# smann95/mpmc

Measured on AMD Instinct MI355X. Metric: MC steps/sec (polarizable, 4096 atoms), higher is better.
Workload: dtype f64; 1 GPU; PCN-61 cell + 416 BSSP H2, 4096 atoms (2016 frozen), polarizable, Jacobi x4, rc 8 A, FH4; energy() incremental (bit-identical to full); n_atoms=4096, n_polarizable=3264, n_atoms_final=4096, n_polarizable_final=3264, walkers=1, parallelism=1 independent walkers, 1 per GPU, collective=none (single walker, no launcher), rccl_ranks=1

## Files before the change

mpmc_amd/csrc/engine.hip:

```cpp
#include "../../include/mpmc_hip.h"

#include <dlfcn.h>
#include <hip/hip_runtime.h>
#include <hip/hip_ext.h>
#include <rccl/rccl.h>

#include <algorithm>
#include <cmath>
#include <cstdarg>
#include <cstdio>
#include <cstring>
#include <functional>
#include <map>
#include <memory>
#include <tuple>
#include <utility>
#include <ctime>
#include <numeric>
#include <atomic>
#include <string>
#include <vector>

#include "device_common.h"
#include "kernels_pair.h"
#include "kernels_disp.h"
#include "kernels_at.h"
#include "kernels_crystal.h"
#include "kernels_vdw.h"
#include "kernels_polar.h"
#include "kernels_exact.h"
#include "kernels_gs.h"
#include "kernels_gs_chain.h"
#include "kernels_resident.h"
#include "kernels_symv.h"
#include "kernels_coef.h"
#include "kernels_volume.h"
#include "kernels_cavity.h"

using namespace mpmc;

static thread_local std::string g_err;
static std::atomic<int> g_ctx_on_device[64];

static int fail(const char *fmt, ...) {
    char buf[1024];
    va_list ap;
    va_start(ap, fmt);
    vsnprintf(buf, sizeof(buf), fmt, ap);
    va_end(ap);
    g_err = buf;
    return -1;
}

#define HIPCHK(expr)                                                                           \
    do {                                                                                       \
        hipError_t e_ = (expr);                                                                \
        if (e_ != hipSuccess) return fail("MPMC_HIP: %s failed: %s (%s:%d)", #expr, hipGetErrorString(e_), \
                                          __FILE__, __LINE__);                                 \
    } while (0)

extern "C" const char *mpmc_hip_last_error(void) { return g_err.c_str(); }
extern "C" int mpmc_hip_abi_version(void) { return MPMC_HIP_ABI_VERSION; }
extern "C" int mpmc_hip_device_count(void) {
    int n = 0;
    if (hipGetDeviceCount(&n) != hipSuccess) return 0;
    return n;
}

template <typename T, bool kPinned>
class HipBuffer {
  public:
    HipBuffer() = default;
    HipBuffer(HipBuffer &&o) noexcept : p_(std::exchange(o.p_, nullptr)), n_(std::exchange(o.n_, 0)) {}
    ~HipBuffer() { reset(); }
    hipError_t alloc(size_t count, unsigned host_flags = hipHostMallocDefault) {
        reset();
        void *p = nullptr;
        hipError_t e;
        if constexpr (kPinned)
            e = hipHostMalloc(&p, count * sizeof(T), host_flags);
        else
            e = hipMalloc(&p, count * sizeof(T));
        if (e == hipSuccess) p_ = static_cast<T *>(p), n_ = count;
        return e;
    }
    void reset() {
        if (p_) {
            if constexpr (kPinned)
                hipHostFree(p_);
            else
// ... 154 lines not shown
    int gs_build_fork = 1;
    int gs_side_waves = 0;
    int rank_view_side = 1;
    int gs_fold_upper = 1;
    int gs_fold_finish = 1;
    int rank_late = 1;
    int resident = 1;
    int res_fold = 16;
    int res_side = 0;
    int sweep_alternate = 1;
    int sweep_nt = -1;
    int sweep_split = -1;
    int fuse_moves = 1;
    int gs_fuse_moves = 1;
    int fuse_field = 1;
    int fuse_recip = 1;
    int split_record = 1;
    int side_moves = 1;
    int res_stamps = 0;
    int sweep_ablate = 0;
    int res_fault = 0;
    int gs_stamps = 0;
    int inv_stamps = 0;
    int gs_ablate = 0;
    int gs_fault_sweep = 0;
    int graph = 0;
};

struct CallState {
    bool do_polar = false;
    bool gs_mode = false;
    bool exact = false;
    bool two_streams = false;
    bool plain_launches = false;
    DirtyBlocks dirty_blocks;
    bool pair_part_valid_before = false;
    bool moves_deferred = false;
    bool moves_in_pair = false;
    bool side_carry = false;
    MoveList side_moves;
    MoveList pair_moves;
    MoveList side_apply;
    bool side_applied = false;
    bool coef_job_valid = false;
    bool coef_job_fork = false;
    CoefJob coef_job;
    bool build_join_pending = false;
    bool rank_on_side = false;
    int gs_sweeps = 0;
    bool gs_used[2] = {false, false};
    std::function<void()> enqueue_side;
    std::function<void()> publish_early;
    bool published = false;
    bool recip_fused = false;
    int recip_chunks = 0;
    int pair_rows_to_sum = 0;
    unsigned res_zero_mask = 0;
    bool split = false;
    bool resident = false;
    bool spec_rank = false;
    bool timed = false;
    int iterations = 0, iter_success = 0;
};

struct TileSum {
    DevBuf<double> part;
    bool valid = false;
};

struct mpmc_hip_ctx {
    int device = 0;
    int num_cus = 256;
    int max_atoms = 0, max_npad = 0;
    int n = 0, npad = 0;
    EngineOptions opt;
    CallState call;
    mpmc_hip_params par;
    bool have_params = false, have_box = false, have_atoms = false;
    double basis[3][3], recip[3][3];
    double pbc_cutoff_in = 0.0, cutoff = 0.0, volume = 0.0, ewald_alpha = 0.0, polar_ewald_alpha = 0.0;
    bool box_ortho = false;
    double coord_max = 0.0;
    unsigned long long config_rev = 1;
    unsigned long long energy_calls = 0;
    bool in_flight = false;
    HipStream stream;
    HipStream stream2;
    HipStream stream3;
    HipEvent ev_fork, ev_join;
    HipEvent ev_rank;
    HipEvent ev_bfork, ev_bjoin;
    HipEvent ev_order;
    DevBuf<double> d_x, d_y, d_z, d_q, d_alpha, d_eps, d_sig, d_molmass;
    DevBuf<int> d_mol, d_flags;
    MoveList pending;
    std::vector<int> dirty_atoms;
    bool all_dirty = true;
    bool staged_copies = false;
    bool main_writes = false;
    SweepView view[2];
    DevBuf<double> d_es, d_mu, d_efind, d_efchg, d_tmp3;
    DevBuf<unsigned long long> d_errmax;
    bool have_polar_result = false;
    SweepView *result_view = nullptr;
    const double *result_mu = nullptr;
    bool results_scattered = true;
// ... 75 lines not shown
    DevBuf<KVec> d_kvec;
    int nk = 0;
    bool kvec_valid = false;
    int kvec_kmax = -1;
    DevBuf<double2> d_sfpart;
    bool recip_part_valid = false;
    DevBuf<double> d_recipsum;
    bool self_valid = false;
    double self_alpha = 0.0;
    DevBuf<KVecF> d_kvecf;
    DevBuf<double2> d_sf;
    int nkf = 0;
    double kvecf_alpha = -1.0;
    int kvecf_kmax = -1;
    bool kvecf_valid = false;
    DevBuf<double> d_rank;
    DevBuf<double> d_rankpart;
    DevBuf<double> d_rank_used;
    DevBuf<unsigned int> d_rankcnt;
    std::vector<double> rank_saved;
    bool perm_ranked = false;
    bool rank_used_valid = false;
    bool force_host_rank = false;
    unsigned long long spec_redos = 0;
    int n_valid = 0;
    int next_mol = 0;
    std::vector<char> slot_valid;
    std::vector<char> slot_polar;
    std::vector<std::pair<int, int>> holes;
    std::vector<int> lrc_dirty_atoms;
    int n_mol_uploaded = 0;
    bool edited = false;
    bool order_stale = false;
    bool resident_off = false;
    long resident_retry_at = 0;
    long resident_backoff = 0;
    bool force_multi_launch = false;
    bool res_attr_set = false;
    unsigned long long resident_calls = 0, resident_fallbacks = 0;
    int graph_mode = 0;
    StepGraph sg;
    int eligible_streak = 0;
    unsigned long long graph_launches = 0;
    double graph_update_s = 0.0, graph_launch_s = 0.0;
    PinnedBuf<int> h_dirty;
    PinnedBuf<double> h_stage;
    size_t stage_used = 0;
    DevBuf<double> d_delta;
    DevBuf<double> d_res;
    PinnedBuf<double> h_res;
    double *h_res_dev = nullptr;
    PinnedBuf<double> h_res2;
    double *h_res2_dev = nullptr;
    PinnedBuf<unsigned long long> h_err;
    PinnedBuf<unsigned> h_gserr;
    PinnedBuf<int> h_order;
    PinnedBuf<double> h_rank;
    PinnedBuf<int> h_perm;
    PinnedBuf<int> h_slotmap;
    std::vector<HipEvent> ev_pool;
    size_t ev_next = 0;
    std::vector<TimeRec> recs;
    HipEvent ev_first, ev_last;
    bool timed = false;
    double host_enqueue_s = 0.0, host_wait_s = 0.0;
};

static DevAtoms dev_atoms(const mpmc_hip_ctx *c) {
    DevAtoms a;
    a.x = c->d_x;
    a.y = c->d_y;
    a.z = c->d_z;
    a.q = c->d_q;
    a.alpha = c->d_alpha;
    a.eps = (c->disp_on || c->rdc_order || c->vdw_on) ? c->d_zero : c->d_eps;
    a.sig = (c->disp_on || c->rdc_order || c->vdw_on) ? c->d_zero : c->d_sig;
    a.molmass = c->d_molmass;
    a.mol = c->d_mol;
    a.flags = c->d_flags;
    a.n = c->n;
    a.npad = c->npad;
    return a;
}

static DevBox dev_box(const mpmc_hip_ctx *c) {
    DevBox b;
    for (int p = 0; p < 3; ++p)
        for (int q = 0; q < 3; ++q) {
            b.b[p][q] = c->basis[p][q];
            b.rb[p][q] = c->recip[p][q];
        }
    b.cutoff = c->cutoff;
    b.volume = c->volume;
    for (int p = 0; p < 3; ++p)
        for (int q = 0; q < 3; ++q) {
            b.fb[p][q] = (float)c->basis[p][q];
            b.frb[p][q] = (float)c->recip[p][q];
        }
    b.rc2_pre = (float)((c->cutoff + 0.01) * (c->cutoff + 0.01));
    b.screen64 = (c->coord_max > kScreen32MaxCoord || !(c->coord_max == c->coord_max)) ? 1 : 0;
    double smax = 0.0, rmax = 0.0;
    for (int q = 0; q < 3; ++q) {
        smax = std::max(smax, std::fabs(c->recip[0][q]) + std::fabs(c->recip[1][q]) + std::fabs(c->recip[2][q]));
        for (int p = 0; p < 3; ++p) rmax = std::max(rmax, std::fabs(c->recip[p][q]));
    }
    const float tie32 = (float)(1.25 * 11.0 * 0x1p-13 * smax);
// ... 246 lines not shown
    HIPCHK(c->d_sig.alloc(np));
    HIPCHK(c->d_molmass.alloc(np));
    HIPCHK(c->d_mol.alloc(np));
    HIPCHK(c->d_flags.alloc(np));
    HIPCHK(c->d_es.alloc(3 * np));
    HIPCHK(c->d_mu.alloc(3 * np));
    HIPCHK(c->d_efind.alloc(3 * np));
    HIPCHK(c->d_efchg.alloc(3 * np));
    HIPCHK(c->d_tmp3.alloc(3 * np));
    HIPCHK(c->d_rank.alloc(np));
    HIPCHK(c->d_rank_used.alloc(np));
    HIPCHK(c->d_rankcnt.alloc(np));
    HIPCHK(c->d_errmax.alloc(256));
    for (SweepView &v : c->view) {
        v.cap = (int)np;
        HIPCHK(v.d_idx.alloc(np));
        HIPCHK(v.d_slot.alloc(np));
        HIPCHK(v.px.alloc(np));
        HIPCHK(v.py.alloc(np));
        HIPCHK(v.pz.alloc(np));
        HIPCHK(v.palpha.alloc(np));
        HIPCHK(v.pflags.alloc(np));
        HIPCHK(v.es.alloc(3 * np));
        HIPCHK(v.mu0.alloc(3 * np));
        HIPCHK(v.mu1.alloc(3 * np));
        HIPCHK(v.munew.alloc(3 * np));
        HIPCHK(v.mupub.alloc(kGsMaxLag * (3 * np + 192)));
        c->gs_qoff = (int)(3 * np + 192);
        HIPCHK(v.y.alloc(3 * np));
        HIPCHK(v.efind.alloc(3 * np));
        HIPCHK(v.tmu0.alloc(3 * np));
        HIPCHK(v.efchg.alloc(3 * np));
        HIPCHK(v.rrms.alloc(np));
        HIPCHK(v.gsflags.alloc(16));
        HIPCHK(hipMemsetAsync(v.gsflags, 0, 16 * sizeof(unsigned), c->stream));
        HIPCHK(v.energy_part.alloc(2 * (np / 64 + 1)));
        for (double *p : {v.mu0.get(), v.mu1.get(), v.munew.get(), v.y.get(), v.efind.get(), v.efchg.get(), v.es.get()})
            HIPCHK(hipMemsetAsync(p, 0, 3 * np * sizeof(double), c->stream));
        HIPCHK(hipMemsetAsync(v.rrms, 0, np * sizeof(double), c->stream));
    }
    const size_t ntile = np / 64;
    HIPCHK(c->d_pairpart.alloc(ntile * ntile * kPairChannels));
    HIPCHK(c->lrc.part.alloc(ntile * ntile));
    HIPCHK(c->d_rankpart.alloc(ntile * ntile));
    const size_t nchunk_max = std::max<size_t>(1, np / 64) + 16;
    HIPCHK(c->d_fieldpart.alloc(nchunk_max * 3 * np));
    HIPCHK(c->d_res.alloc(R_COUNT));
    HIPCHK(c->h_res.alloc(R_COUNT + 1, hipHostMallocMapped));
    c->h_res[R_COUNT] = 0.0;
    HIPCHK(hipHostGetDevicePointer((void **)&c->h_res_dev, c->h_res, 0));
    HIPCHK(c->h_res2.alloc(R_COUNT + 1, hipHostMallocMapped));
    memset(c->h_res2, 0, (R_COUNT + 1) * sizeof(double));
    HIPCHK(hipHostGetDevicePointer((void **)&c->h_res2_dev, c->h_res2, 0));
    HIPCHK(c->h_err.alloc(1));
    HIPCHK(c->h_gserr.alloc(2));
    HIPCHK(c->h_rank.alloc(np));
    HIPCHK(c->h_perm.alloc(np));
    HIPCHK(c->h_slotmap.alloc(np));
    HIPCHK(c->h_dirty.alloc(kMaxDirty));
    HIPCHK(c->h_stage.alloc(3 * 4096));
    c->ev_pool.resize(2 * 512);
    for (auto &e : c->ev_pool) HIPCHK(hipEventCreate(e.out()));
    HIPCHK(hipEventCreate(c->ev_first.out()));
    HIPCHK(hipEventCreate(c->ev_last.out()));
    HIPCHK(hipMemsetAsync(c->d_res, 0, R_COUNT * sizeof(double), c->stream));
    HIPCHK(hipStreamSynchronize(c->stream));
    if (device < 64) ++g_ctx_on_device[device];
    *out = owner.release();
    return 0;
}

static void graph_destroy(mpmc_hip_ctx *c);

extern "C" void mpmc_hip_destroy(mpmc_hip_ctx *c) {
    if (!c) return;
    if (getenv("MPMC_HIP_HOST_PROFILE") && c->energy_calls)
        fprintf(stderr, "MPMC_HIP host profile: %llu energy() calls (%llu as graph), enqueue %.1f us, wait %.1f us per call\n",
                c->energy_calls, c->graph_launches, 1e6 * c->host_enqueue_s / c->energy_calls,
                1e6 * c->host_wait_s / c->energy_calls);
    if (getenv("MPMC_HIP_HOST_PROFILE") && c->graph_launches)
        fprintf(stderr, "MPMC_HIP graph steps: node updates %.1f us, launch %.1f us per step\n",
                1e6 * c->graph_update_s / c->graph_launches, 1e6 * c->graph_launch_s / c->graph_launches);
    hipSetDevice(c->device);
    hipStreamSynchronize(c->stream);
    hipStreamSynchronize(c->stream2);
    hipStreamSynchronize(c->stream3);
    graph_destroy(c);
    if (c->device < 64) --g_ctx_on_device[c->device];
    delete c;
}

static void positions_unknown(mpmc_hip_ctx *c) {
    c->pair_part_valid = c->field_part_valid = c->disp.valid = c->rdc.valid = c->at.valid = false;
    c->rep.valid = c->vdw.valid = false;
}
static void params_or_grid_changed(mpmc_hip_ctx *c) {
    c->pair_part_valid = c->field_part_valid = c->disp.valid = c->rdc.valid = false;
    c->rep.valid = c->vdw.valid = false;
}
static void box_changed(mpmc_hip_ctx *c) {
    c->lrc.valid = c->disp_lrc.valid = c->rdc_static.valid = c->rep_lrc.valid = c->vdw_lrc.valid = false;
    c->cav_pos_valid = c->cav_occ_valid = false;
    c->cav_open = -1;
}
static void atoms_replaced(mpmc_hip_ctx *c) {
    c->lrc.valid = c->disp.valid = c->disp_lrc.valid = c->at.valid = c->rdc.valid = c->rdc_static.valid = false;
// ... 1791 lines not shown
                hipGraph_t graph = nullptr;
                ok = (hipStreamEndCapture(c->stream, &graph) == hipSuccess) && rc == 0 && graph != nullptr;
                if (ok) ok = graph_finish_capture(c, graph);
                else if (graph) hipGraphDestroy(graph);
            }
            if (ok) {
                c->sg.valid = true;
                c->sg.rev = c->config_rev;
                c->sg.iterations = c->call.iterations;
                c->sg.result_view = c->result_view;
                c->sg.result_mu = c->result_mu;
                c->sg.psweep = c->psweep;
                c->sg.energy_part = c->energy_part;
                c->sg.energy_nt = c->energy_nt;
                c->sg.recip_chunks = c->call.recip_chunks;
                c->sg.res_zero_mask = c->call.res_zero_mask;
                c->sg.pair_rows_to_sum = c->call.pair_rows_to_sum;
                HIPCHK(hipGraphLaunch(c->sg.exec, c->stream));
                ++c->graph_launches;
                issued = true;
            } else {
                (void)hipGetLastError();
                graph_destroy(c);
                c->opt.graph = 0;
                c->pending = saved;
                c->call = CallState();
                collect_dirty_blocks(c);
            }
        }
    } else {
        c->eligible_streak = 0;
    }
    if (!issued && enqueue_direct(c)) return -1;
    c->staged_copies = false;
    c->main_writes = false;
    clock_gettime(CLOCK_MONOTONIC, &ts1);
    c->host_enqueue_s += (ts1.tv_sec - ts0.tv_sec) + 1e-9 * (ts1.tv_nsec - ts0.tv_nsec);
    c->dirty_atoms.clear();
    c->all_dirty = false;
    c->in_flight = true;
    return 0;
}

static int wait_sequence(volatile double *seq, double want, hipStream_t stream) {
    for (unsigned long long spins = 0; spins < 2000000000ull; ++spins) {
        if (*seq == want) return 0;
        if ((spins & 0xfffffull) == 0xfffffull && hipStreamQuery(stream) != hipErrorNotReady) break;
        __builtin_ia32_pause();
    }
    HIPCHK(hipStreamSynchronize(stream));
    return 0;
}

static int wait_record(mpmc_hip_ctx *c) {
    const double want = (double)c->energy_calls;
    if (wait_sequence(c->h_res + R_COUNT, want, c->stream)) return -1;
    return c->call.split ? wait_sequence(c->h_res2 + R_COUNT, want, c->stream2) : 0;
}

static int repeat_call(mpmc_hip_ctx *c, bool &flag) {
    flag = true;
    begin_call(c);
    const int rc = enqueue_direct(c);
    flag = false;
    return rc ? -1 : wait_record(c);
}

extern "C" int mpmc_hip_energy_end(mpmc_hip_ctx *c, mpmc_hip_result *out) {
    if (!c || !out) return fail("MPMC_HIP: energy: null argument");
    if (!c->in_flight) return fail("MPMC_HIP: energy_end: no evaluation in flight");
    c->in_flight = false;
    memset(out, 0, sizeof(*out));
    const mpmc_hip_params &P = c->par;
    timespec ts1, ts2;
    clock_gettime(CLOCK_MONOTONIC, &ts1);
    if (wait_record(c)) return -1;
    if (c->call.spec_rank && c->h_res[R_GS_ERR] == 0.0 && c->h_res[R_RANKCHG] != 0.0) {
        ++c->spec_redos;
        if (repeat_call(c, c->force_host_rank)) return -1;
    }
    if (c->call.resident && c->h_res[R_GS_ERR] != 0.0) {
        ++c->resident_fallbacks;
        c->resident_off = true;
        c->resident_backoff = c->resident_backoff ? std::min(2 * c->resident_backoff, 1L << 20) : 4096;
        c->resident_retry_at = (long)c->energy_calls + c->resident_backoff;
        c->view[0].resP_armed = false;
        if (repeat_call(c, c->force_multi_launch)) return -1;
    }
    clock_gettime(CLOCK_MONOTONIC, &ts2);
    c->host_wait_s += (ts2.tv_sec - ts1.tv_sec) + 1e-9 * (ts2.tv_nsec - ts1.tv_nsec);
    const bool do_polar = c->call.do_polar, timed_call = c->call.timed;
    const int polar_iterations = c->call.iterations;
    const int iter_success = c->call.exact ? (c->h_res[R_RRMS] != 0.0 ? 1 : 0) : c->call.iter_success;
    if (c->call.exact) {
        c->chol_done = true;
        c->chol_failed = iter_success != 0;
    }
    const int gs_err = (int)c->h_res[R_GS_ERR];
    c->h_gserr[0] = gs_err & 1;
    c->h_gserr[1] = (gs_err >> 1) & 1;
    const bool gs_timeout = gs_err != 0;
    if (gs_timeout) {
        unsigned dbg[8] = {0};
        const SweepView &gv = c->view[c->h_gserr[1] ? 1 : 0];
        hipMemcpy(dbg, gv.gsflags, sizeof(dbg), hipMemcpyDeviceToHost);
        return fail("MPMC_HIP: persistent Gauss-Seidel kernel gave up waiting on a hand-off (spin limit) in view %d: "
                    "workgroup %u thread %u addr-lo 0x%x; mu_new-lo 0x%x",
                    c->h_gserr[1] ? 1 : 0, dbg[2], dbg[3], dbg[4], (unsigned)((unsigned long long)gv.mupub.get() & 0xffffffffu));
    }
    HIPCHK(hipGetLastError());
    c->timed = timed_call;
    c->stage_used = 0;

    double r[R_COUNT];
    for (int k = 0; k < R_COUNT; ++k) r[k] = (c->call.split && ((kSideSlots >> k) & 1u)) ? c->h_res2[k] : c->h_res[k];
    const double rd = c->disp_on     ? (r[R_RD_PAIR] + r[R_LRC]) + (r[R_DISP] + r[R_DISP_LRC])
                      : c->rdc_order ? (r[R_RD_PAIR] + r[R_LRC]) + ((r[R_DISP] + r[R_RDC_SELF]) + r[R_DISP_LRC])
                      : c->vdw_on    ? (r[R_RD_PAIR] + r[R_LRC]) + (r[R_DISP] + r[R_DISP_LRC])
                                     : r[R_RD_PAIR] + r[R_LRC];
    const double real = r[R_ES_REAL] - r[R_ES_INTRA];
    const bool ewald = !P.rd_only && !P.wolf;
    const double recip = ewald ? r[R_RECIP] * (4.0 * kPI / c->volume) : 0.0;
    const double self = ewald ? r[R_SELF] : 0.0;
    const double coul = P.rd_only ? 0.0 : real + recip + self;
    const double upol = do_polar ? r[R_UPOL] : 0.0;
    out->rd_energy = rd;
    out->es_real = P.rd_only ? 0.0 : real;
    out->es_recip = recip;
    out->es_self = self;
    out->coulombic_energy = coul;
    out->polarization_energy = upol;
    out->energy = rd + coul + upol;
    c->three_body = c->at_on ? r[R_AT] : 0.0;
    if (c->at_on) out->energy += c->three_body;
    c->vdw_energy = (c->vdw_on && !P.rd_only) ? ((r[R_VDW] - c->vdw_e_iso) + 0.0) + r[R_VDW_LRC] : 0.0;
    if (c->vdw_on) out->energy += c->vdw_energy;
    c->vdw_terms[0] = (c->vdw_on && !P.rd_only) ? r[R_VDW] : 0.0;
    c->vdw_terms[1] = (c->vdw_on && !P.rd_only) ? c->vdw_e_iso : 0.0;
    c->vdw_terms[2] = (c->vdw_on && !P.rd_only) ? r[R_VDW_LRC] : 0.0;
    c->vdw_terms[3] = c->vdw_on ? r[R_DISP] : 0.0;
    c->vdw_terms[4] = c->vdw_on ? r[R_DISP_LRC] : 0.0;
    c->close_contacts = c->autoreject_scale != 0.0 ? (long long)r[R_CONTACTS] : 0;
    out->dipole_rrms = (do_polar && !c->call.exact) ? r[R_RRMS] : 0.0;
    out->volume = c->volume;
    out->cutoff = c->cutoff;
    out->ewald_alpha = c->ewald_alpha;
    out->polar_ewald_alpha = c->polar_ewald_alpha;
    out->polar_iterations = polar_iterations;
    out->iter_success = iter_success;
    out->n_atoms = c->n_valid;
    out->status = std::isfinite(out->energy) ? 0 : 1;
    return 0;
}

extern "C" int mpmc_hip_download_dipoles(mpmc_hip_ctx *c, double *mu, double *ef_static, double *ef_induced,
                                         double *ef_induced_change) {
    if (!c || !c->have_atoms) return fail("MPMC_HIP: download_dipoles: no configuration");
    if (!c->have_polar_result) return fail("MPMC_HIP: download_dipoles: no polarization energy evaluated yet");
    HIPCHK(hipSetDevice(c->device));
    if (ensure_static_field(c)) return -1;
    if (complete_pending_sweep(c)) return -1;
    if (!c->results_scattered) {
        SweepView *V = c->result_view;
        hipLaunchKernelGGL(scatter_results_kernel, dim3((c->npad + 255) / 256), dim3(256), 0, c->stream, c->npad,
                           V->d_slot, c->result_mu, V->efind, V->efchg, c->d_mu, c->d_efind, c->d_efchg);
        HIPCHK(hipStreamSynchronize(c->stream));
        c->results_scattered = true;
    }
// ... 425 lines not shown
```

mpmc_amd/csrc/engine_polar.inc:

```
static constexpr bool kSweepSplitAuto = false;

static int launch_coef_job(mpmc_hip_ctx *c, const DevBox &bx) {
    if (!c->call.coef_job_valid) return 0;
    c->call.coef_job_valid = false;
    const CoefJob &cj = c->call.coef_job;
    hipLaunchKernelGGL(update_coef_moves_kernel, dim3(cj.nt, cj.dm.n), dim3(64), 0, c->stream, cj.pa, bx, cj.damp, cj.dm,
                       cj.ntld, cj.C, cj.m, cj.gx, cj.gy, cj.gz, cj.slot_of_atom, cj.px, cj.py, cj.pz);
    if (c->call.coef_job_fork) hipEventRecord(c->ev_fork, c->stream);
    return 0;
}

static int launch_field(mpmc_hip_ctx *c, const DevAtoms &a, const DevBox &bx) {
    const mpmc_hip_params &P = c->par;
    ScopedTimer t(c, T_FIELD);
    FieldParams fp;
    fp.wolf_alpha = P.polar_wolf_alpha;
    fp.cutoffterm = 0.0;
    const int ntile = c->npad / 64;
    int nchunk = std::max(1, std::min(ntile, 4096 / ntile));
    int chunk = round_up((c->npad + nchunk - 1) / nchunk, 64);
    nchunk = (c->npad + chunk - 1) / chunk;
    fp.chunk = chunk;
    const int mode = P.polar_ewald ? kFieldEwald : (!P.polar_wolf ? kFieldBare : (P.polar_wolf_alpha == 0.0 ? kFieldWolf0 : kFieldWolfA));
    const int key = mode * 1000003 + chunk;
// ... 298 lines not shown
                c->call.build_join_pending = true;
            }
            if (istamps) {
                --c->opt.inv_stamps;
                std::vector<unsigned long long> h(nwg * 4);
                HIPCHK(hipStreamSynchronize(st));
                HIPCHK(hipMemcpy(h.data(), istamps, h.size() * sizeof(unsigned long long), hipMemcpyDeviceToHost));
                unsigned long long t0 = ~0ull, t3 = 0;
                double ph[3] = {0, 0, 0}, phmax[3] = {0, 0, 0}, start_max = 0;
                int live = 0;
                for (size_t g = 0; g < nwg; ++g) {
                    if (!h[4 * g + 3]) continue;
                    t0 = std::min(t0, h[4 * g]);
                }
                for (size_t g = 0; g < nwg; ++g) {
                    if (!h[4 * g + 3]) continue;
                    ++live;
                    t3 = std::max(t3, h[4 * g + 3]);
                    start_max = std::max(start_max, (double)(h[4 * g] - t0) * 0.01);
                    for (int k = 0; k < 3; ++k) {
                        const double d = (double)(h[4 * g + k + 1] - h[4 * g + k]) * 0.01;
                        ph[k] += d;
                        phmax[k] = std::max(phmax[k], d);
                    }
                }
                fprintf(stderr, "INV_STAMPS waves %d, %d live workgroups of %zu (lists %d %d %d, full %d): span %.2f us, last start +%.2f us; "
                                "mean (max) us: loads %.2f (%.2f), expansion %.2f (%.2f), substitution %.2f (%.2f)\n",
                        waves, live, nwg, gb.inv.n, gb.own.n, nsingle, full ? 1 : 0, (double)(t3 - t0) * 0.01, start_max, ph[0] / std::max(live, 1),
                        phmax[0], ph[1] / std::max(live, 1), phmax[1], ph[2] / std::max(live, 1), phmax[2]);
            }
        }
        v.M_epoch = v.C_epoch;
        v.M_call = c->energy_calls;
    }
    if (want_matrix) {
        if (ensure_view_matrix(v)) return -1;
        if (can_update && v.A_valid) {
            if (nd > 0)
                hipLaunchKernelGGL(update_amatrix_kernel, dim3(v.nvpad / 128, nd), dim3(64), 0, st, pa, bx,
                                   c->par.polar_damp, dl, v.A, 3 * v.nvpad);
        } else {
            hipLaunchKernelGGL(build_amatrix_kernel, dim3(v.nvpad / 128, v.nvpad / kARows), dim3(64), 0, st, pa, bx,
                               c->par.polar_damp, v.A, 3 * v.nvpad);
            v.A_valid = true;
        }
    } else {
        v.A_valid = false;
    }
    return 0;
}

template <int MODE>
static int launch_sweep(mpmc_hip_ctx *c, SweepView &v, const DevBox &bx, const double *mu_in, double *out,
                        const SweepParams &sp, int timer_class, const double *mu_final = nullptr) {
    const int nvpad = v.nvpad, lda = 3 * nvpad;
    if (v.C_valid) {
        const int nt = std::max(1, (v.nv + kCoefTile - 1) / kCoefTile);
        if (ensure_coef_scratch(v, nt)) return -1;
        CoefFinish fin;
        fin.alpha = v.palpha;
        fin.flags = v.pflags;
        fin.mu_in = mu_in;
        fin.es = v.es;
        fin.ef_induced = v.efind;
        fin.out = out;
        fin.rrms = v.rrms;
        fin.errmax = c->d_errmax;
        fin.mu_final = mu_final;
        fin.energy_part = v.energy_part;
        fin.tmu0 = v.tmu0;
        fin.sp = sp;
        size_t half_plane = 0;
        {
            const int ntiles = nt * (nt + 1) / 2;
            const bool split = c->opt.sweep_split > 0 || (c->opt.sweep_split < 0 && kSweepSplitAuto && nt > 21 && ntiles < 8 * c->num_cus);
            half_plane = split ? 2 * (3 * (size_t)kCoefTile * nt) * (size_t)nt : 0;
            const dim3 g(split ? 16 * ((ntiles + 7) / 8) : ntiles), b(64 * kCoefWaves);
            const size_t tile_bytes = (size_t)nt * (nt + 1) / 2 * kCoefTile * kCoefTile * sizeof(double2);
            const bool sweep_nt = c->opt.sweep_nt > 0 || (c->opt.sweep_nt < 0 && tile_bytes > ((size_t)224 << 20));
            void (*kern)(const double2 *, int, int, const double *, const double *, const double *, const double *, DevBox,
                         double *, double *, int, size_t) =
                c->box_ortho ? (sweep_nt ? pair_sweep_kernel<1, 1> : pair_sweep_kernel<1, 0>)
                             : (sweep_nt ? pair_sweep_kernel<0, 1> : pair_sweep_kernel<0, 0>);
            if (split)
                kern = c->box_ortho ? (sweep_nt ? pair_sweep_kernel<1, 1, 0, 1> : pair_sweep_kernel<1, 0, 0, 1>)
                                    : (sweep_nt ? pair_sweep_kernel<0, 1, 0, 1> : pair_sweep_kernel<0, 0, 0, 1>);
            if (c->opt.sweep_ablate == 1) kern = pair_sweep_kernel<1, 0, 1>;
            if (c->opt.sweep_ablate == 2) kern = pair_sweep_kernel<1, 0, 2>;
            if (c->opt.sweep_ablate) half_plane = 0;
            HIPCHK(launch_timed(c, timer_class, kern, g, b, 0, c->stream, (const double2 *)v.C, nt, v.ntld,
                                (const double *)v.px, (const double *)v.py, (const double *)v.pz, mu_in, bx, v.Srow, v.Zcol,
                                c->opt.sweep_alternate ? (c->sweep_parity++ & 1) : 0, half_plane));
        }
        {
            ScopedTimer t2(c, T_OTHER);
            hipLaunchKernelGGL(pair_finish_kernel<MODE>, dim3(nt), dim3(64 * kCoefFinishGroups), 0, c->stream, nt, v.Srow,
                               v.Zcol, fin, half_plane);
        }
        c->energy_part = v.energy_part;
        c->energy_nt = nt;
        return 0;
    }
    c->energy_nt = 0;
    if (c->opt.symmetric && (nvpad >= 2048 || c->opt.symmetric > 1)) {
        if (ensure_sym_scratch(v)) return -1;
        {
            ScopedTimer t(c, timer_class);
            const dim3 g(nvpad / kSymChunkAtoms, nvpad / kSymRowAtoms);
            const int rev = (c->opt.sym_mode & 1) ? (c->sweep_parity++ & 1) : 0;
            if (c->opt.sym_mode & 2)
                hipLaunchKernelGGL(symv_kernel<1>, g, dim3(64), 0, c->stream, v.A, lda, nvpad, mu_in, v.Srow, v.Zcol, rev,
                                   v.nv);
            else
                hipLaunchKernelGGL(symv_kernel<0>, g, dim3(64), 0, c->stream, v.A, lda, nvpad, mu_in, v.Srow, v.Zcol, rev,
                                   v.nv);
        }
        ScopedTimer t2(c, T_OTHER);
        hipLaunchKernelGGL(symv_finish_kernel<MODE>, dim3(nvpad / 64), dim3(1024), 0, c->stream, nvpad, v.Srow, v.Zcol,
                           v.palpha, v.pflags, mu_in, v.es, v.efind, out, v.rrms, c->d_errmax, sp);
    } else {
        ScopedTimer t(c, timer_class);
        hipLaunchKernelGGL(sweep_kernel<MODE>, dim3(nvpad), dim3(64), 0, c->stream, v.A, lda, nvpad, v.palpha,
                           v.pflags, mu_in, v.es, v.efind, out, v.rrms, c->d_errmax, sp);
    }
    return 0;
}

static bool defer_last_sweep(const mpmc_hip_ctx *c, const SweepView &v) {
    const mpmc_hip_params &P = c->par;
    if (!c->opt.pair_coef || !v.C_valid) return false;
    if (P.polar_zodid || P.polar_gs || P.polar_gs_ranked || P.polar_palmo || P.polar_sor || P.polar_esor || P.polar_rrms)
        return false;
    if (P.polar_precision != 0.0 || P.polar_gamma != 1.0 || P.polar_max_iter < 2) return false;
    const int nt = std::max(1, (v.nv + kCoefTile - 1) / kCoefTile);
    return nt * (nt + 1) / 2 + nt > c->num_cus;
}

static int complete_pending_sweep(mpmc_hip_ctx *c) {
    if (c->psweep.sweeps.empty()) return 0;
    PendingSweep p;
    std::swap(p, c->psweep);
    HIPCHK(hipSetDevice(c->device));
    for (const PendingSweep::One &s : p.sweeps)
        if (launch_sweep<kSweepJacobi>(c, *p.view, p.bx, s.mu_in, s.mu_out, s.sp, T_SWEEP)) return -1;
    return 0;
}

static void (*chain_kernel_of(int ortho))(GsChain) { return ortho ? gs_chain_kernel<1> : gs_chain_kernel<0>; }

static bool gs_uses_chain(const mpmc_hip_ctx *c) { return c->opt.pair_coef != 0 && c->opt.persistent_gs != 0; }

struct GsFinishArgs {
    double w_new, w_old;
    int want_rrms, err_slot;
    double *mu_out;
};
static int launch_gs_sweep(mpmc_hip_ctx *c, SweepView &v, const DevAtoms &a, const DevBox &bx, const double *mu_old,
                           const GsFinishArgs *fin = nullptr, bool *finished = nullptr) {
    if (finished) *finished = false;
    const int nvpad = v.nvpad, lda = 3 * nvpad;
    (void)a;
    ++c->call.gs_sweeps;
    if (gs_uses_chain(c) && v.C_valid) {
        const int nt = std::max(1, (v.nv + kCoefTile - 1) / kCoefTile);
        if (ensure_coef_scratch(v, nt)) return -1;
        const bool fold_upper = c->opt.gs_fold_upper && fin && c->opt.gs_fold_finish && !c->opt.gs_ablate;
        {
            ScopedTimer tu(c, T_OTHER);
            const dim3 g(nt * (nt + 1) / 2), b(64 * kCoefWaves);
            const int rev = c->opt.sweep_alternate ? (c->sweep_parity++ & 1) : 0;
            if (c->box_ortho)
                hipLaunchKernelGGL(pair_upper_kernel<1>, g, b, 0, c->stream, v.C, nt, v.ntld, v.px, v.py, v.pz, mu_old, bx, v.Srow, rev,
                                   fold_upper ? nt : 0, v.mupub, v.gsflags, c->gs_qoff);
            else
                hipLaunchKernelGGL(pair_upper_kernel<0>, g, b, 0, c->stream, v.C, nt, v.ntld, v.px, v.py, v.pz, mu_old, bx, v.Srow, rev,
                                   fold_upper ? nt : 0, v.mupub, v.gsflags, c->gs_qoff);
            if (!fold_upper)
                hipLaunchKernelGGL(pair_upper_finish_kernel, dim3(nvpad / 64), dim3(64 * kCoefFinishGroups), 0, c->stream, nt,
                                   v.Srow, v.y, 1, v.mupub, v.gsflags, c->gs_qoff);
        }
        GsChain gp;
        gp.C = v.C;
        gp.ntld = v.ntld;
        gp.nb = nt;
        gp.px = v.px;
        gp.py = v.py;
        gp.pz = v.pz;
        gp.alpha = v.palpha;
// ... 363 lines not shown
        const double scale = (!P.polar_sor && !P.polar_esor) ? P.polar_gamma : 1.0;
        hipLaunchKernelGGL(init_view_kernel, dim3(V->nvpad / 64), dim3(64 * kFieldGroups), 0, c->stream, V->nv,
                           V->nvpad, V->d_idx, V->palpha, c->d_fieldpart, c->es_slots, c->npad, scale, V->es, mu_in,
                           V->efind, V->efchg, V->rrms, c->d_errmax,
                           (chain_mode || rp.ok) ? c->view[0].gsflags : (unsigned *)nullptr,
                           chain_mode ? c->view[1].gsflags : (unsigned *)nullptr,
                           rp.ok ? V->respub : (double *)nullptr, P.polar_max_iter, (size_t)3 * V->nvpad);
    }

    int iteration_counter = 0;
    bool ranked_active = false;
    const bool defer = !rp.ok && defer_last_sweep(c, *V);
    c->psweep.drop();
    if (rp.ok) {
        if (launch_resident(c, *V, bx, rp, want_rrms)) return -1;
        iteration_counter = P.polar_max_iter;
        mu_in = V->mu1;
    } else if (!P.polar_zodid) {
        bool keep_iterating = true;
        while (keep_iterating) {
            iteration_counter++;
            const int nvpad = V->nvpad;
            const dim3 gvec((nvpad + 255) / 256), bvec(256);
            if (iteration_counter >= kMAX_ITERATION_COUNT && P.polar_precision != 0.0) {
                hipLaunchKernelGGL(fallback_dipoles_kernel, gvec, bvec, 0, c->stream, nvpad, V->palpha, V->es, mu_in,
                                   V->efchg);
                *iter_success = 1;
                break;
            }
            double w_new = 1.0, w_old = 0.0;
            if (P.polar_sor) {
                w_new = P.polar_gamma;
                w_old = 1.0 - P.polar_gamma;
            } else if (P.polar_esor) {
                w_old = std::exp(-P.polar_gamma * iteration_counter);
                w_new = 1.0 - w_old;
            }
            const double *palmo_mu = mu_in;
            if (!gs) {
                SweepParams sp;
                sp.w_new = w_new;
                sp.w_old = w_old;
                sp.want_rrms = want_rrms;
                sp.want_err = P.polar_precision > 0.0;
                sp.err_slot = iteration_counter;
                sp.skip_sums = (P.polar_precision == 0.0 && iteration_counter < P.polar_max_iter) ? 1 : 0;
                const int mid = (P.polar_max_iter + 1) / 2;
                if (defer) {
                    const bool odd = P.polar_max_iter & 1;
                    sp.skip_sums = 1;
                    if (odd && iteration_counter == P.polar_max_iter - mid) sp.energy_mode |= kEnergyStoreSums;
                    if (iteration_counter == mid) sp.energy_mode |= kEnergyMid | (odd ? kEnergyPrevSums : 0);
                }
                if (defer && (iteration_counter == P.polar_max_iter || (iteration_counter > mid && c->call.published))) {
                    PendingSweep &ps = c->psweep;
                    ps.view = V;
                    ps.bx = bx;
                    PendingSweep::One one;
                    one.mu_in = mu_in;
                    one.mu_out = mu_out;
                    one.sp = sp;
                    ps.sweeps.push_back(one);
                } else if (launch_sweep<kSweepJacobi>(c, *V, bx, mu_in, mu_out, sp, T_SWEEP)) {
                    return -1;
                }
                if (c->call.enqueue_side && (iteration_counter == c->opt.side_after || P.polar_max_iter < c->opt.side_after)) c->call.enqueue_side();
                if (defer && iteration_counter == mid && c->call.publish_early) {
                    if (c->call.enqueue_side) c->call.enqueue_side();
                    c->call.publish_early();
                }
            } else {
                GsFinishArgs gfa;
                gfa.w_new = w_new;
                gfa.w_old = w_old;
                gfa.want_rrms = (int)want_rrms;
                gfa.err_slot = (P.polar_precision > 0.0) ? iteration_counter : -1;
                gfa.mu_out = mu_out;
                bool finished = false;
                if (launch_gs_sweep(c, *V, a, bx, mu_in, &gfa, &finished)) return -1;
                const bool planar = gs_uses_chain(c) && V->C_valid;
                if (!finished)
                hipLaunchKernelGGL(gs_finish_kernel, gvec, bvec, 0, c->stream, nvpad, V->palpha, V->pflags, mu_in,
                                   (const double *)(planar ? V->mupub : V->munew), planar ? 1 : 0, V->y, w_new, w_old,
                                   (int)want_rrms, iteration_counter, mu_out, planar ? V->munew : (double *)nullptr,
                                   V->efind, V->rrms, c->d_errmax);
                palmo_mu = V->munew;
            }

            if (P.polar_precision == 0.0) {
                keep_iterating = (iteration_counter != P.polar_max_iter);
            } else {
                HIPCHK(hipMemcpyAsync(c->h_err, c->d_errmax + iteration_counter, sizeof(unsigned long long),
                                      hipMemcpyDeviceToHost, c->stream));
                HIPCHK(hipStreamSynchronize(c->stream));
                double emax;
                memcpy(&emax, c->h_err, sizeof(double));
                const double allowed = P.polar_precision * P.polar_precision * kDEBYE2SKA * kDEBYE2SKA;
                keep_iterating = (emax > allowed);
            }

            if (P.polar_palmo && !keep_iterating) {
                SweepParams sp;
                sp.w_new = 1.0;
                sp.w_old = 0.0;
                sp.want_rrms = 0;
                sp.want_err = 0;
                sp.err_slot = 0;
                sp.skip_sums = 0;
                if (launch_sweep<kSweepPalmo>(c, *V, bx, palmo_mu, V->efchg, sp, T_PALMO, gs ? V->munew : mu_out)) return -1;
            }

            std::swap(mu_in, mu_out);

            if (ranked && !rank_enqueued) {
                enqueue_rank();
                if (rank_rc) return -1;
            }
            if (ranked && keep_iterating && !ranked_active) {
                ScopedTimer t(c, T_OTHER);
                if (spec_rank) {
                    hipStreamWaitEvent(c->stream, c->ev_rank, 0);
                } else {
// ... 97 lines not shown
```

mpmc_amd/csrc/kernels_coef.h:

```cpp
#pragma once
#include "device_common.h"
#include "kernels_polar.h"

namespace mpmc {

constexpr int kGsArmRegions = 4;
constexpr int kCoefTile = 64;
constexpr int kCoefWaves = 4;
constexpr int kCoefSteps = kCoefTile / kCoefWaves;
__host__ __device__ __forceinline__ size_t coef_tile_index(int ti, int tj, int ntld) { return (size_t)tj * ntld + ti; }

template <int ORTHO>
__device__ __forceinline__ void image_displacement(const DevBox &bx, double dx, double dy, double dz, double &ox,
                                                   double &oy, double &oz) {
    double i0, i1, i2;
    {
#pragma clang fp contract(off)
        if (ORTHO) {
            i0 = bx.rb[0][0] * dx;
            i1 = bx.rb[1][1] * dy;
            i2 = bx.rb[2][2] * dz;
        } else {
            i0 = bx.rb[0][0] * dx;
            i0 = i0 + bx.rb[1][0] * dy;
// ... 147 lines not shown
                                                                double *pz) {
    update_coef_moves_body(blockIdx.x, blockIdx.y, threadIdx.x, blockIdx.x == 0 && blockIdx.y == 0, a, bx, damp, dm, ntld, C,
                           m, gx, gy, gz, slot_of_atom, px, py, pz);
}

struct CoefJob {
    DevAtoms pa;
    double damp;
    DirtyMoves dm;
    int nt, ntld;
    double2 *C;
    MoveList m;
    double *gx, *gy, *gz;
    const int *slot_of_atom;
    double *px, *py, *pz;
};
template <int MODE>
__global__ __launch_bounds__(64 * kFieldWaves) void field_coef_kernel(DevAtoms a, DevBox bx, FieldParams fp, DirtyBlocks sel,
                                                                       double *__restrict__ part, CoefJob cj) {
    if (blockIdx.z == 2) {
        const int u = ((int)blockIdx.y * (int)gridDim.x + (int)blockIdx.x) * kFieldWaves + ((int)threadIdx.x >> 6);
        const int bxi = u % cj.nt, byi = u / cj.nt;
        if (byi < cj.dm.n)
            update_coef_moves_body(bxi, byi, threadIdx.x & 63, u == 0, cj.pa, bx, cj.damp, cj.dm, cj.ntld, cj.C, cj.m, cj.gx,
                                   cj.gy, cj.gz, cj.slot_of_atom, cj.px, cj.py, cj.pz);
        return;
    }
    static_field_body<MODE>(a, bx, fp, sel, part, cj.m);
}

__device__ __forceinline__ void upper_tile_of(int t, int nt, int &ti, int &tj) {
    const float b = 2.0f * (float)nt + 1.0f;
    int r = (int)((b - sqrtf(b * b - 8.0f * (float)t)) * 0.5f);
    r = max(0, min(r, nt - 1));
    while (r > 0 && r * nt - r * (r - 1) / 2 > t) --r;
    while ((r + 1) * nt - (r + 1) * r / 2 <= t) ++r;
    ti = r;
    tj = r + (t - (r * nt - r * (r - 1) / 2));
}

struct CoefFinish {
    const double *alpha;
    const int *flags;
    const double *mu_in;
    const double *es;
    double *ef_induced;
    double *out;
    double *rrms;
    unsigned long long *errmax;
    const double *mu_final;
    double *energy_part;
    double *tmu0;
    SweepParams sp;
};

template <int MODE>
__device__ __forceinline__ void coef_epilogue(const CoefFinish &f, int t, int i, int lane, const double s[3], double al,
                                              int fl, const double old[3], const double es[3], const double aux[3],
                                              double m_out[3], double e_out[3], bool want_sums = true,
                                              bool store = true) {
#pragma clang fp contract(off)
    const bool valid = fl & kValid;
    double e_i = 0.0, r_i = 0.0, emax_i = 0.0;
    m_out[0] = m_out[1] = m_out[2] = 0.0;
    e_out[0] = e_out[1] = e_out[2] = 0.0;
    if ((MODE == kSweepJacobi && (al == 0.0 || !valid)) || (MODE == kSweepPalmo && !valid)) {
        if (store) {
#pragma unroll
            for (int p = 0; p < 3; ++p) {
                f.out[3 * i + p] = 0.0;
                if (MODE == kSweepJacobi) f.ef_induced[3 * i + p] = 0.0;
            }
            if (MODE == kSweepJacobi && f.sp.want_rrms) f.rrms[i] = 0.0;
        }
    } else if (MODE == kSweepJacobi) {
        double d2 = 0.0, n2 = 0.0, emax = 0.0, m[3];
#pragma unroll
        for (int p = 0; p < 3; ++p) {
            const double e = -s[p];
            const double nw = al * (es[p] + e);
            if (store) f.ef_induced[3 * i + p] = e;
            e_out[p] = e;
            m[p] = f.sp.w_new * nw + f.sp.w_old * old[p];
            m_out[p] = m[p];
            if (store) f.out[3 * i + p] = m[p];
            const double d = nw - old[p];
            d2 += d * d;
            n2 += nw * nw;
            emax = fmax(emax, d * d);
        }
        if (f.sp.want_rrms) {
            double rr = sqrt(d2 / n2);
            if (!isfinite(rr)) rr = 0.0;
            if (store) f.rrms[i] = rr;
            r_i = rr;
        }
        emax_i = emax;
        e_i = m[0] * es[0] + m[1] * es[1] + m[2] * es[2];
    } else {
        double m[3], dc[3];
#pragma unroll
        for (int p = 0; p < 3; ++p) {
            dc[p] = -aux[p] - s[p];
            f.out[3 * i + p] = dc[p];
            m[p] = old[p];
        }
// ... 53 lines not shown
            const int u = u0 + k * kCoefFinishGroups;
            const bool on = u < nterm;
            const int ux = on ? u : g;
            const int uu = ux >= nt ? ux - nt : ux;
            const double *p = (uu < nt - t) ? Srow + (size_t)(t + uu) * ncol : Zcol + (size_t)(uu - (nt - t)) * ncol;
            p += 192 * t + lane + (ux >= nt ? half_plane : 0);
            v[k][0] = on ? p[0] : 0.0;
            v[k][1] = on ? p[64] : 0.0;
            v[k][2] = on ? p[128] : 0.0;
        }
#pragma unroll
        for (int k = 0; k < 4; ++k) {
            s0 += v[k][0];
            s1 += v[k][1];
            s2 += v[k][2];
        }
    }
    part[g][0][lane] = s0;
    part[g][1][lane] = s1;
    part[g][2][lane] = s2;
    __syncthreads();
    if (g != 0) return;
    double s[3];
#pragma unroll
    for (int p = 0; p < 3; ++p) {
        double acc = 0.0;
#pragma unroll
        for (int k = 0; k < kCoefFinishGroups; ++k) acc += part[k][p][lane];
        s[p] = acc;
    }
    double m_new[3], e_new[3];
    const int emode = (MODE == kSweepJacobi) ? f.sp.energy_mode : 0;
    coef_epilogue<MODE>(f, t, i, lane, s, al, fl, old, es, aux, m_new, e_new, !f.sp.skip_sums && !(emode & kEnergyMid));
    if (emode) {
#pragma clang fp contract(off)
        if (emode & kEnergyStoreSums) {
#pragma unroll
            for (int p = 0; p < 3; ++p) f.tmu0[3 * i + p] = s[p];
        }
        if (emode & kEnergyMid) {
            double e_i = 0.0;
            if ((fl & kValid) && al != 0.0) {
                if (!(emode & kEnergyPrevSums)) {
#pragma unroll
                    for (int p = 0; p < 3; ++p) sk[p] = s[p];
                }
                e_i = m_new[0] * es[0] + m_new[1] * es[1] + m_new[2] * es[2];
                e_i -= (m_new[0] - old[0]) * sk[0] + (m_new[1] - old[1]) * sk[1] + (m_new[2] - old[2]) * sk[2];
            }
            e_i = wave_sum(e_i);
            if (lane == 0) {
                f.energy_part[2 * t] = e_i;
                f.energy_part[2 * t + 1] = 0.0;
            }
        }
    }
}

template <int ORTHO, int TIGHT, int PREMUL, int STEPS>
__device__ __forceinline__ void tile_part_product(const double2 (&c)[STEPS], int l, int base, double xi, double yi,
                                                  double zi, double mix, double miy, double miz, const double2 *jxy,
                                                  const double2 *jzm, const double2 *jmm, const DevBox &bx, double &sx,
                                                  double &sy, double &sz, double &zx, double &zy, double &zz) {
    sx = sy = sz = zx = zy = zz = 0.0;
#pragma unroll
    for (int k = 0; k < STEPS; ++k) {
        const int jj = (l + base + k) & 63;
        const double2 pa = jxy[jj], pb = jzm[jj], pm = jmm[jj];
        double dx, dy, dz;
        image_displacement<ORTHO>(bx, xi - pa.x, yi - pa.y, zi - pb.x, dx, dy, dz);
        const double c3 = c[k].x, c5m = PREMUL ? c[k].y : -3.0 * c[k].y;
        const double wj = c5m * fma(dz, pm.y, fma(dy, pm.x, dx * pb.y));
        sx = fma(wj, dx, fma(c3, pb.y, sx));
        sy = fma(wj, dy, fma(c3, pm.x, sy));
        sz = fma(wj, dz, fma(c3, pm.y, sz));
        if (k > 0) {
            zx = wave_rotate_down(zx);
            zy = wave_rotate_down(zy);
            zz = wave_rotate_down(zz);
        }
        const double wi = c5m * fma(dz, miz, fma(dy, miy, dx * mix));
        zx = fma(wi, dx, fma(c3, mix, zx));
        zy = fma(wi, dy, fma(c3, miy, zy));
        zz = fma(wi, dz, fma(c3, miz, zz));
        if (TIGHT) __builtin_amdgcn_sched_barrier(0);
    }
}
template <int ORTHO, int TIGHT = 0, int PREMUL = 0>
__device__ __forceinline__ void tile_quarter_product(const double2 (&c)[kCoefSteps], int l, int w, double xi, double yi,
                                                     double zi, double mix, double miy, double miz, const double2 *jxy,
                                                     const double2 *jzm, const double2 *jmm, const DevBox &bx, double &sx,
                                                     double &sy, double &sz, double &zx, double &zy, double &zz) {
    tile_part_product<ORTHO, TIGHT, PREMUL, kCoefSteps>(c, l, kCoefSteps * w, xi, yi, zi, mix, miy, miz, jxy, jzm, jmm, bx, sx, sy,
                                                        sz, zx, zy, zz);
}


template <int ORTHO, int NT = 1, int ABLATE = 0, int SPLIT = 0>
__global__ __launch_bounds__(64 * kCoefWaves) void pair_sweep_kernel(const double2 *__restrict__ C, int nt, int ntld,
                                                                       const double *__restrict__ x,
                                                                       const double *__restrict__ y,
                                                                       const double *__restrict__ z,
                                                                       const double *__restrict__ mu, DevBox bx,
                                                                       double *__restrict__ Srow,
                                                                       double *__restrict__ Zcol, int rev,
                                                                       size_t half_plane) {
// ... 195 lines not shown
```

Before: 14130 MC steps/s.

## Stream per-block U_pol shares to mapped host memory and fold on host

At the mid-iteration energy point, each coefficient sweep block writes its partial polarization energy plus a sequence stamp straight into mapped pinned host memory. The host polls all stamps, then folds the partials in a fixed IEEE-order tree so the result matches the device reduction. This replaces the separate publish/reduce step and its record-completion wait. The path is gated to split, non-resident, non-exact configurations, and the rest of the result record is zeroed in this mode. It adds many system-scope fences and host PCIe polling.

```diff
diff --git a/mpmc_amd/csrc/engine.hip b/mpmc_amd/csrc/engine.hip
--- a/mpmc_amd/csrc/engine.hip
+++ b/mpmc_amd/csrc/engine.hip
@@ -36,6 +36,7 @@
 #include "kernels_coef.h"
 #include "kernels_volume.h"
 #include "kernels_cavity.h"
+#include "record_fold.h"
 
 using namespace mpmc;
 
@@ -296,6 +297,8 @@
     std::function<void()> enqueue_side;
     std::function<void()> publish_early;
     bool published = false;
+    bool host_record = false;
+    int host_nt = 0;
     bool recip_fused = false;
     int recip_chunks = 0;
     int pair_rows_to_sum = 0;
@@ -477,6 +480,9 @@
     double *h_res_dev = nullptr;
     PinnedBuf<double> h_res2;
     double *h_res2_dev = nullptr;
+    PinnedBuf<mpmc::RecordShare> h_share;
+    double *h_share_dev = nullptr;
+    double main_rec[R_COUNT] = {0.0};
     PinnedBuf<unsigned long long> h_err;
     PinnedBuf<unsigned> h_gserr;
     PinnedBuf<int> h_order;
@@ -829,6 +835,9 @@
     HIPCHK(c->h_res2.alloc(R_COUNT + 1, hipHostMallocMapped));
     memset(c->h_res2, 0, (R_COUNT + 1) * sizeof(double));
     HIPCHK(hipHostGetDevicePointer((void **)&c->h_res2_dev, c->h_res2, 0));
+    HIPCHK(c->h_share.alloc(np / 64 + 1, hipHostMallocMapped));
+    memset(c->h_share, 0, c->h_share.size() * sizeof(mpmc::RecordShare));
+    HIPCHK(hipHostGetDevicePointer((void **)&c->h_share_dev, c->h_share, 0));
     HIPCHK(c->h_err.alloc(1));
     HIPCHK(c->h_gserr.alloc(2));
     HIPCHK(c->h_rank.alloc(np));
@@ -2726,9 +2735,41 @@
     return 0;
 }
 
+static int wait_shares(mpmc_hip_ctx *c, double want, double *upol) {
+    const volatile mpmc::RecordShare *sh = c->h_share;
+    const int nt = c->call.host_nt;
+    if (nt < 1 || (size_t)nt > c->h_share.size()) return fail("MPMC_HIP: internal: host record of %d blocks", nt);
+    int missing = nt;
+    for (unsigned long long spins = 0; spins < 2000000000ull; ++spins) {
+        missing = mpmc::missing_shares(sh, nt, want);
+        if (!missing) break;
+        if ((spins & 0xfffffull) == 0xfffffull && hipStreamQuery(c->stream) != hipErrorNotReady) break;
+        __builtin_ia32_pause();
+    }
+    if (missing) {
+        HIPCHK(hipStreamSynchronize(c->stream));
+        int first = -1;
+        missing = mpmc::missing_shares(sh, nt, want, &first);
+        if (missing)
+            return fail("MPMC_HIP: the result record is incomplete: %d of %d blocks did not hand over their share of U_pol "
+                        "(first: block %d, stamp %.17g, call %.17g)", missing, nt, first, (double)sh[first].stamp, want);
+    }
+    __atomic_thread_fence(__ATOMIC_ACQUIRE);
+    *upol = mpmc::fold_upol(&sh[0].value, nt, (int)(sizeof(mpmc::RecordShare) / sizeof(double)));
+    return 0;
+}
+
 static int wait_record(mpmc_hip_ctx *c) {
     const double want = (double)c->energy_calls;
-    if (wait_sequence(c->h_res + R_COUNT, want, c->stream)) return -1;
+    if (c->call.host_record) {
+        double upol = 0.0;
+        if (wait_shares(c, want, &upol)) return -1;
+        for (int k = 0; k < R_COUNT; ++k) c->main_rec[k] = 0.0;
+        c->main_rec[R_UPOL] = upol;
+    } else {
+        if (wait_sequence(c->h_res + R_COUNT, want, c->stream)) return -1;
+        for (int k = 0; k < R_COUNT; ++k) c->main_rec[k] = c->h_res[k];
+    }
     return c->call.split ? wait_sequence(c->h_res2 + R_COUNT, want, c->stream2) : 0;
 }
 
@@ -2749,11 +2790,11 @@
     timespec ts1, ts2;
     clock_gettime(CLOCK_MONOTONIC, &ts1);
     if (wait_record(c)) return -1;
-    if (c->call.spec_rank && c->h_res[R_GS_ERR] == 0.0 && c->h_res[R_RANKCHG] != 0.0) {
+    if (c->call.spec_rank && c->main_rec[R_GS_ERR] == 0.0 && c->main_rec[R_RANKCHG] != 0.0) {
         ++c->spec_redos;
         if (repeat_call(c, c->force_host_rank)) return -1;
     }
-    if (c->call.resident && c->h_res[R_GS_ERR] != 0.0) {
+    if (c->call.resident && c->main_rec[R_GS_ERR] != 0.0) {
         ++c->resident_fallbacks;
         c->resident_off = true;
         c->resident_backoff = c->resident_backoff ? std::min(2 * c->resident_backoff, 1L << 20) : 4096;
@@ -2765,12 +2806,12 @@
     c->host_wait_s += (ts2.tv_sec - ts1.tv_sec) + 1e-9 * (ts2.tv_nsec - ts1.tv_nsec);
     const bool do_polar = c->call.do_polar, timed_call = c->call.timed;
     const int polar_iterations = c->call.iterations;
-    const int iter_success = c->call.exact ? (c->h_res[R_RRMS] != 0.0 ? 1 : 0) : c->call.iter_success;
+    const int iter_success = c->call.exact ? (c->main_rec[R_RRMS] != 0.0 ? 1 : 0) : c->call.iter_success;
     if (c->call.exact) {
         c->chol_done = true;
         c->chol_failed = iter_success != 0;
     }
-    const int gs_err = (int)c->h_res[R_GS_ERR];
+    const int gs_err = (int)c->main_rec[R_GS_ERR];
     c->h_gserr[0] = gs_err & 1;
     c->h_gserr[1] = (gs_err >> 1) & 1;
     const bool gs_timeout = gs_err != 0;
@@ -2787,7 +2828,7 @@
     c->stage_used = 0;
 
     double r[R_COUNT];
-    for (int k = 0; k < R_COUNT; ++k) r[k] = (c->call.split && ((kSideSlots >> k) & 1u)) ? c->h_res2[k] : c->h_res[k];
+    for (int k = 0; k < R_COUNT; ++k) r[k] = (c->call.split && ((kSideSlots >> k) & 1u)) ? c->h_res2[k] : c->main_rec[k];
     const double rd = c->disp_on     ? (r[R_RD_PAIR] + r[R_LRC]) + (r[R_DISP] + r[R_DISP_LRC])
                       : c->rdc_order ? (r[R_RD_PAIR] + r[R_LRC]) + ((r[R_DISP] + r[R_RDC_SELF]) + r[R_DISP_LRC])
                       : c->vdw_on    ? (r[R_RD_PAIR] + r[R_LRC]) + (r[R_DISP] + r[R_DISP_LRC])
diff --git a/mpmc_amd/csrc/engine_polar.inc b/mpmc_amd/csrc/engine_polar.inc
--- a/mpmc_amd/csrc/engine_polar.inc
+++ b/mpmc_amd/csrc/engine_polar.inc
@@ -374,7 +374,8 @@
 
 template <int MODE>
 static int launch_sweep(mpmc_hip_ctx *c, SweepView &v, const DevBox &bx, const double *mu_in, double *out,
-                        const SweepParams &sp, int timer_class, const double *mu_final = nullptr) {
+                        const SweepParams &sp, int timer_class, const double *mu_final = nullptr,
+                        bool host_share = false) {
     const int nvpad = v.nvpad, lda = 3 * nvpad;
     if (v.C_valid) {
         const int nt = std::max(1, (v.nv + kCoefTile - 1) / kCoefTile);
@@ -392,6 +393,11 @@
         fin.energy_part = v.energy_part;
         fin.tmu0 = v.tmu0;
         fin.sp = sp;
+        if (host_share) {
+            fin.host_share = c->h_share_dev;
+            fin.host_seq = (double)c->energy_calls;
+            c->call.host_nt = nt;
+        }
         size_t half_plane = 0;
         {
             const int ntiles = nt * (nt + 1) / 2;
@@ -456,6 +462,15 @@
     if (P.polar_precision != 0.0 || P.polar_gamma != 1.0 || P.polar_max_iter < 2) return false;
     const int nt = std::max(1, (v.nv + kCoefTile - 1) / kCoefTile);
     return nt * (nt + 1) / 2 + nt > c->num_cus;
+}
+
+static bool host_record_ok(const mpmc_hip_ctx *c, const SweepView &v) {
+    const CallState &k = c->call;
+    if (!k.split || k.exact || k.gs_mode || k.spec_rank || k.resident || k.gs_used[0] || k.gs_used[1]) return false;
+    if (c->par.polar_rrms || c->par.polar_gs_ranked) return false;
+    if (c->autoreject_scale != 0.0 || c->vdw_on) return false;
+    const int nt = std::max(1, (v.nv + kCoefTile - 1) / kCoefTile);
+    return (size_t)nt <= c->h_share.size();
 }
 
 static int complete_pending_sweep(mpmc_hip_ctx *c) {
@@ -925,6 +940,8 @@
                     if (odd && iteration_counter == P.polar_max_iter - mid) sp.energy_mode |= kEnergyStoreSums;
                     if (iteration_counter == mid) sp.energy_mode |= kEnergyMid | (odd ? kEnergyPrevSums : 0);
                 }
+                const bool to_host = defer && iteration_counter == mid && c->call.publish_early && !c->call.published &&
+                                     !c->call.build_join_pending && host_record_ok(c, *V);
                 if (defer && (iteration_counter == P.polar_max_iter || (iteration_counter > mid && c->call.published))) {
                     PendingSweep &ps = c->psweep;
                     ps.view = V;
@@ -934,13 +951,18 @@
                     one.mu_out = mu_out;
                     one.sp = sp;
                     ps.sweeps.push_back(one);
-                } else if (launch_sweep<kSweepJacobi>(c, *V, bx, mu_in, mu_out, sp, T_SWEEP)) {
+                } else if (launch_sweep<kSweepJacobi>(c, *V, bx, mu_in, mu_out, sp, T_SWEEP, nullptr, to_host)) {
                     return -1;
                 }
                 if (c->call.enqueue_side && (iteration_counter == c->opt.side_after || P.polar_max_iter < c->opt.side_after)) c->call.enqueue_side();
                 if (defer && iteration_counter == mid && c->call.publish_early) {
                     if (c->call.enqueue_side) c->call.enqueue_side();
-                    c->call.publish_early();
+                    if (to_host) {
+                        c->call.published = true;
+                        c->call.host_record = true;
+                    } else {
+                        c->call.publish_early();
+                    }
                 }
             } else {
                 GsFinishArgs gfa;
diff --git a/mpmc_amd/csrc/kernels_coef.h b/mpmc_amd/csrc/kernels_coef.h
--- a/mpmc_amd/csrc/kernels_coef.h
+++ b/mpmc_amd/csrc/kernels_coef.h
@@ -223,6 +223,8 @@
     double *energy_part;
     double *tmu0;
     SweepParams sp;
+    double *host_share = nullptr;
+    double host_seq = 0.0;
 };
 
 template <int MODE>
@@ -382,6 +384,12 @@
             if (lane == 0) {
                 f.energy_part[2 * t] = e_i;
                 f.energy_part[2 * t + 1] = 0.0;
+                if (f.host_share) {
+                    volatile double *h = f.host_share + 2 * t;
+                    h[0] = e_i;
+                    __threadfence_system();
+                    h[1] = f.host_seq;
+                }
             }
         }
     }
diff --git a/mpmc_amd/csrc/record_fold.h b/mpmc_amd/csrc/record_fold.h
--- /dev/null
+++ b/mpmc_amd/csrc/record_fold.h
@@ -0,0 +1,44 @@
+#pragma once
+
+#if defined(__FAST_MATH__)
+#error "record_fold.h: the fold is a fixed sequence of IEEE additions; build without -ffast-math"
+#endif
+
+namespace mpmc {
+
+struct RecordShare {
+    double value;
+    double stamp;
+};
+
+constexpr int kFoldLanes = 64;
+
+inline double fold_upol(const volatile double *part, int nt, int stride = 1) {
+#if defined(__clang__)
+#pragma clang fp contract(off) reassociate(off)
+#endif
+    double a[kFoldLanes], b[kFoldLanes];
+    for (int l = 0; l < kFoldLanes; ++l) {
+        double acc = 0.0;
+        for (int t = l; t < nt; t += kFoldLanes) acc = acc + part[(long)t * stride];
+        a[l] = acc;
+    }
+    for (int off = kFoldLanes / 2; off > 0; off >>= 1) {
+        for (int l = 0; l < kFoldLanes; ++l) b[l] = a[l] + a[l ^ off];
+        for (int l = 0; l < kFoldLanes; ++l) a[l] = b[l];
+    }
+    return -0.5 * a[0];
+}
+
+inline int missing_shares(const volatile RecordShare *share, int nt, double want, int *first_missing = nullptr) {
+    int missing = 0;
+    for (int t = 0; t < nt; ++t) missing += (share[t].stamp != want) ? 1 : 0;
+    if (first_missing) {
+        *first_missing = -1;
+        for (int t = nt - 1; t >= 0 && missing; --t)
+            if (share[t].stamp != want) *first_missing = t;
+    }
+    return missing;
+}
+
+}
```

Result: slower. 13660 MC steps/s (-3.3%).
